# Superjie13/StereoTracking

Hardware: AMD Instinct MI355X
Metric: stereo frame-pairs/sec @1280x720 D=192 (higher is better)
Workload: dtype f32; 1 GPU; configs[1]: batch=8 synthetic 1280x720 stereo pairs per GPU, D=192, full YOLOX-s two-branch backbone+PAFPN+head, cost volume at 1/4 res (48 levels) + 2 3x3 aggregation convs + soft-argmin, decode+NMS, per-box depth; global_batch=8, inflight_contexts=4, distinct_input_batches=4, gpu_max_hw_queues=4, hip_force_dev_kernarg=1, parallelism=single process, no process group (no collective in the step), collectives_issued=0, tuning_plan=configs/tuning/mi355x.json, max_det=1000, detections_overflow=False

## Files before the change

include/stereotrack.h:

```cpp
#ifndef STEREOTRACK_H_
#define STEREOTRACK_H_

#include <stddef.h>
#include <stdint.h>

#ifdef __cplusplus
extern "C" {
#endif

#define ST_VERSION 430

enum {
  ST_OK = 0,
  ST_ERR_INVALID = -1,
  ST_ERR_HIP = -2,
  ST_ERR_STATE = -3,
  ST_ERR_WORKSPACE = -4,
  ST_ERR_NOTFOUND = -5
};

typedef void* st_stream_t;

int st_version(void);
const char* st_last_error(void);

typedef struct StConvDesc {
  const float* in_dev;
  int N, Hi, Wi, Cin, in_ld, in_off;
  const float* wgt_dev;
  const float* bias_dev;
  int Cout, KH, KW, stride, pad;
  float* out1_dev;
  int out1_ld, out1_off, split;
  float* out2_dev;
  int out2_ld, out2_off;
  float* up_dev;
  int up_ld, up_off;
  const float* res_dev;
  int res_ld, res_off;
  float post_scale;
  int act;
  const float* wgt_wino_dev;
} StConvDesc;

int st_conv2d_nhwc(const StConvDesc* d, st_stream_t stream);
int st_conv2d_nhwc_variant(const StConvDesc* d, st_stream_t stream, int variant);
size_t st_wino_packed_floats(int Cout, int Cin);
int st_wino_pack_weights(const float* packed_wgt_host, int Cout, int Cin, float* out_host);
int st_conv3x3_wino_group(const StConvDesc* descs, int n, st_stream_t stream);

int st_conv1x1_chain(const StConvDesc* a, const StConvDesc* b, st_stream_t stream);
size_t st_front_frag_floats(int Cout, int Cin);
int st_front_pack_frags(const float* packed_wgt_host, int Cout, int Cin, float* out_host);
int st_conv3x3s2_csp_front(const StConvDesc* a, const StConvDesc* ms, const StConvDesc* c1, const float* frag_ms_dev,
                           const float* frag_c1_dev, st_stream_t stream);
size_t st_csp_tail_frag_floats(void);
int st_csp_tail_pack_frags(const float* packed_wgt_host, float* out_host);
int st_conv3x3_csp_tail(const StConvDesc* conv2, const StConvDesc* fin, const float* frag_fin_dev, st_stream_t stream);
size_t st_conv_packed_floats(int Cout, int Cin, int KH, int KW);
int st_conv_pack_weights(const float* w, const float* conv_bias,
                         const float* bn_gamma, const float* bn_beta,
                         const float* bn_mean, const float* bn_var,
                         double bn_eps, int Cout, int Cin, int KH, int KW,
                         float* wgt_out, float* bias_out);

int st_focus_pack(const float* img_nchw_dev, int N, int C, int H, int W,
                  float* out_nhwc_dev, st_stream_t stream);

size_t st_stem_packed_floats(int Cout);
int st_stem_pack_weights(const float* w, const float* conv_bias,
                         const float* bn_gamma, const float* bn_beta,
                         const float* bn_mean, const float* bn_var,
                         double bn_eps, int Cout, int used_planes, float* wgt_out, float* bias_out);
int st_stem_focus_conv(const float* img_nchw_dev, int N, int H, int W, int used_planes, const float* wgt_dev,
                       const float* bias_dev, int Cout, float* out_nhwc_dev, int out_ld, int out_off,
                       int act , st_stream_t stream);
int st_stem_focus_conv_u8(const unsigned char* const* frames_u8_dev_ptrs_host, int N, int h, int w, int H, int W,
                          float pad_value, const float* wgt_dev, const float* bias_dev, int Cout, float* out_dev,
                          int out_ld, int out_off, int act, st_stream_t stream);

int st_pack_raw_inputs(const unsigned char* img_u8_dev, const unsigned short* disp_u16_dev, int N, int h, int w,
                       int H, int W, float img_pad, float* img_out_dev, float* disp_postp_out_dev,
                       float* disp_mask_out_dev, st_stream_t stream);
int st_pack_raw_frames(const unsigned char* const* frames_u8_dev_ptrs_host, int N, int h, int w, int H, int W,
                       float img_pad, float* img_out_dev, st_stream_t stream);
int st_resize_planes(const void* in_dev, int P, int h, int w, int interleaved, void* out_dev, int h2, int w2,
                     int elem_bytes, int bilinear, st_stream_t stream);

int st_spp_pool(const float* x_dev, int x_ld, int x_off, int N, int H, int W, int C,
                float* out_dev, int out_ld, int out_off, st_stream_t stream);

typedef struct StDetector StDetector;

typedef struct StDetectorConfig {
  int struct_size;
  float widen_factor;
  float deepen_factor;
  int num_classes;
  int batch;
// ... 398 lines not shown
```

stereotracking_amd/_lib.py:

```python
import ctypes as C
import os

import torch

_HERE = os.path.dirname(os.path.abspath(__file__))
LIB_PATH = os.path.join(_HERE, 'lib', 'libstereotrack_hip.so')

ST_OK = 0
_ERR_NAMES = {-1: 'ST_ERR_INVALID', -2: 'ST_ERR_HIP', -3: 'ST_ERR_STATE', -4: 'ST_ERR_WORKSPACE',
              -5: 'ST_ERR_NOTFOUND'}


class StError(RuntimeError):
    """A libstereotrack_hip call returned a non-zero status."""


class StConvDesc(C.Structure):
    _fields_ = [
        ('in_dev', C.c_void_p),
        ('N', C.c_int), ('Hi', C.c_int), ('Wi', C.c_int), ('Cin', C.c_int), ('in_ld', C.c_int), ('in_off', C.c_int),
        ('wgt_dev', C.c_void_p), ('bias_dev', C.c_void_p),
        ('Cout', C.c_int), ('KH', C.c_int), ('KW', C.c_int), ('stride', C.c_int), ('pad', C.c_int),
        ('out1_dev', C.c_void_p), ('out1_ld', C.c_int), ('out1_off', C.c_int), ('split', C.c_int),
        ('out2_dev', C.c_void_p), ('out2_ld', C.c_int), ('out2_off', C.c_int),
# ... 70 lines not shown
        [(n, C.c_void_p) for n in ('gt_rows', 'pred_rows', 'ignore_rows', 'frame_gt_off', 'frame_pred_off',
                                   'frame_ignore_off', 'frame_ws_off', 'class_table', 'ws')] + [('ws_bytes', C.c_size_t)] + \
        [(n, C.c_void_p) for n in ('gt_keep', 'pred_keep', 'status')]


class StTrackletArgs(C.Structure):
    _fields_ = [(n, C.c_int) for n in ('struct_size', 'num_rows', 'num_out_rows', 'num_tracks', 'first', 'count',
                                       'num_groups', 'max_rows')] + \
        [(n, C.c_void_p) for n in ('rows', 'row_out_off', 'row_gap', 'trk_out_off', 'trk_order', 'trk_len_scale', 'ws')] + \
        [('ws_bytes', C.c_size_t), ('out_rows', C.c_void_p), ('status', C.c_void_p), ('phase_ticks', C.c_void_p)]


class StStreamTick(C.Structure):
    _fields_ = [('struct_size', C.c_int), ('streams', C.c_int), ('chunk', C.c_int), ('num_chunks', C.c_int),
                ('max_dets', C.c_int), ('det_rows', C.c_int), ('stream_of_slot', C.c_void_p), ('frame_ids', C.c_void_p)]


class StHeadPredLevel(C.Structure):
    _fields_ = [('cls_dev', C.c_void_p), ('cls_ld', C.c_int), ('cls_off', C.c_int),
                ('reg_dev', C.c_void_p), ('reg_ld', C.c_int), ('reg_off', C.c_int),
                ('wgt_cls_dev', C.c_void_p), ('bias_cls_dev', C.c_void_p),
                ('wgt_reg_dev', C.c_void_p), ('bias_reg_dev', C.c_void_p),
                ('out_dev', C.c_void_p), ('M', C.c_int)]


class StDecodeDesc(C.Structure):
    _fields_ = [
        ('struct_size', C.c_int), ('batch', C.c_int), ('num_levels', C.c_int),
        ('level_h', C.c_int * 4), ('level_w', C.c_int * 4), ('level_stride', C.c_int * 4),
        ('level_offset', C.c_size_t * 4),
        ('score_thr', C.c_float), ('iou_thr', C.c_float), ('max_det', C.c_int),
        ('scale_x', C.c_float), ('scale_y', C.c_float), ('pad_left', C.c_float), ('pad_top', C.c_float),
        ('ori_w', C.c_float), ('ori_h', C.c_float), ('nms_mask_rows', C.c_int), ('num_classes', C.c_int),
        ('single_label', C.c_int),
    ]


_vp, _i, _f, _sz = C.c_void_p, C.c_int, C.c_float, C.c_size_t
_PROTOS = {
    'st_version': (C.c_int, []),
    'st_head_row_floats': (_i, [_i]),
    'st_png_unfilter': (_i, [_vp, _i, _i, _i, _vp]),
    'st_stem_focus_conv_u8': (_i, [_vp, _i, _i, _i, _i, _i, _f, _vp, _vp, _i, _vp, _i, _i, _i, _vp]),
    'st_detector_forward_raw': (_i, [_vp, _vp, _i, _i, _f, _vp, _vp, _sz, _vp, _vp]),
    'st_detector_forward_phase0_raw': (_i, [_vp, _vp, _vp, _i, _i, _f, _vp, _sz, _vp]),
    'st_pack_raw_frames': (_i, [_vp, _i, _i, _i, _i, _i, _f, _vp, _vp]),
    'st_resize_planes': (_i, [_vp, _i, _i, _i, _i, _vp, _i, _i, _i, _i, _vp]),
    'st_detector_set_split': (_i, [_vp, _i]),
    'st_split_instances_available': (_i, []),
    'st_volume_agg3d': (_i, [_vp, _vp, _i, _i, _i, _i, _vp, _f, _i, _vp]),
    'st_last_error': (C.c_char_p, []),
    'st_conv2d_nhwc': (_i, [C.POINTER(StConvDesc), _vp]),
    'st_conv2d_nhwc_variant': (_i, [C.POINTER(StConvDesc), _vp, _i]),
    'st_conv3x3_wino_group': (_i, [C.POINTER(StConvDesc), _i, _vp]),
    'st_head_pred': (_i, [C.POINTER(StHeadPredLevel), _i, _i, _vp]),
    'st_detector_op_owner': (_i, [_vp, _i, _vp, _vp]),
    'st_conv1x1_chain': (_i, [C.POINTER(StConvDesc), C.POINTER(StConvDesc), _vp]),
    'st_front_frag_floats': (_sz, [_i, _i]),
    'st_front_pack_frags': (_i, [_vp, _i, _i, _vp]),
    'st_conv3x3s2_csp_front': (_i, [C.POINTER(StConvDesc), C.POINTER(StConvDesc), C.POINTER(StConvDesc), _vp, _vp, _vp]),
    'st_csp_tail_frag_floats': (_sz, []),
    'st_csp_tail_pack_frags': (_i, [_vp, _vp]),
    'st_conv3x3_csp_tail': (_i, [C.POINTER(StConvDesc), C.POINTER(StConvDesc), _vp, _vp]),
    'st_conv_packed_floats': (_sz, [_i, _i, _i, _i]),
    'st_wino_packed_floats': (_sz, [_i, _i]),
    'st_wino_pack_weights': (_i, [_vp, _i, _i, _vp]),
    'st_conv_pack_weights': (_i, [_vp, _vp, _vp, _vp, _vp, _vp, C.c_double, _i, _i, _i, _i, _vp, _vp]),
    'st_focus_pack': (_i, [_vp, _i, _i, _i, _i, _vp, _vp]),
    'st_stem_packed_floats': (_sz, [_i]),
    'st_stem_pack_weights': (_i, [_vp, _vp, _vp, _vp, _vp, _vp, C.c_double, _i, _i, _vp, _vp]),
    'st_stem_focus_conv': (_i, [_vp, _i, _i, _i, _i, _vp, _vp, _i, _vp, _i, _i, _i, _vp]),
    'st_pack_raw_inputs': (_i, [_vp, _vp, _i, _i, _i, _i, _i, _f, _vp, _vp, _vp, _vp]),
    'st_spp_pool': (_i, [_vp, _i, _i, _i, _i, _i, _i, _vp, _i, _i, _vp]),
    'st_detector_create': (_i, [C.POINTER(StDetectorConfig), C.POINTER(_vp)]),
    'st_detector_destroy': (_i, [_vp]),
    'st_detector_num_params': (_i, [_vp]),
    'st_detector_param_info': (_i, [_vp, _i, C.c_char_p, _i, C.POINTER(C.c_int64), C.POINTER(_i)]),
    'st_detector_set_param': (_i, [_vp, C.c_char_p, _vp, C.c_int64]),
    'st_detector_finalize': (_i, [_vp]),
    'st_detector_workspace_bytes': (_sz, [_vp]),
    'st_detector_head_floats': (_sz, [_vp]),
    'st_detector_num_levels': (_i, [_vp]),
    'st_detector_level_info': (_i, [_vp, _i, C.POINTER(_i), C.POINTER(_i), C.POINTER(_i), C.POINTER(_sz)]),
    'st_detector_forward': (_i, [_vp, _vp, _vp, _vp, _sz, _vp, _vp]),
    'st_detector_forward_phase': (_i, [_vp, _i, _vp, _vp, _vp, _vp, _sz, _vp, _vp]),
    'st_detector_macs': (C.c_double, [_vp]),
    'st_detector_set_timing': (_i, [_vp, _i]),
    'st_detector_num_ops': (_i, [_vp]),
    'st_detector_op_times': (_i, [_vp, _i, _vp, _vp, _vp, _vp, _vp]),
    'st_detector_autotune': (_i, [_vp, _vp, _sz, _vp, _vp, _i]),
    'st_conv_variant_name': (C.c_char_p, [_i]),
    'st_conv_variant_signature': (C.c_char_p, [_i]),
    'st_detector_get_tuning': (_i, [_vp, _vp, _i]),
    'st_detector_set_tuning': (_i, [_vp, _vp, _i]),
    'st_detector_op_desc': (_i, [_vp, _i, C.c_char_p, _i]),
    'st_detector_tap': (_i, [_vp, C.c_char_p, _vp, C.POINTER(_vp), C.POINTER(_i), C.POINTER(_i),
                             C.POINTER(_i), C.POINTER(_i), C.POINTER(_i)]),
    'st_decode_nms_workspace_bytes': (_sz, [C.POINTER(StDecodeDesc)]),
    'st_lapjv_extended': (_i, [_vp, _i, _i, C.c_double, _vp, _vp]),
    'st_tracker_create': (_i, [C.POINTER(StTrackerConfig), C.POINTER(_vp)]),
    'st_tracker_destroy': (_i, [_vp]),
    'st_tracker_reset': (_i, [_vp]),
    'st_tracker_track': (_i, [_vp, _i, _vp, _i, _vp, _vp, _i, C.POINTER(_i)]),
    'st_tracker_track_records': (_i, [_vp, _vp, _vp, _i, _i, _i, _vp, _vp, _i, _vp]),
    'st_tracker_cmc_needed': (_i, [_vp, _i, _i]),
    'st_tracker_track_cmc': (_i, [_vp, _i, _vp, _i, _vp, _vp, _vp, _i, C.POINTER(_i)]),
# ... 102 lines not shown
```

stereotracking_amd/csrc/conv_igemm.hip:

```cpp
#include <algorithm>

#include <type_traits>

#include "st_common.h"

namespace st {

typedef float f32x16 __attribute__((ext_vector_type(16)));
typedef float f32x4 __attribute__((ext_vector_type(4)));
typedef unsigned int u32x4 __attribute__((ext_vector_type(4)));

struct ConvKArgs {
  const float* in;
  const float* wgt;
  const float* bias;
  float* out1;
  float* out2;
  float* up;
  const float* res;
  int Hi, Wi, Cin, in_ld, in_off;
  int Ho, Wo, HoWo, Cout;
  int KH, KW, stride, pad;
  int K, Kpad, M;
  unsigned in_bytes, wgt_bytes;
  int out1_ld, out1_off, split;
  int out2_ld, out2_off;
  int up_ld, up_off;
  int res_ld, res_off;
  float post_scale;
  int act;
  int n_tiles;
};

constexpr int BK = 32;
constexpr int LDK = 36;

__device__ __forceinline__ float silu_f32(float v) {
  return v * __builtin_amdgcn_rcpf(1.0f + __expf(-v));
}

template <int TM, int TN>
__device__ __forceinline__ void conv_epilogue(const ConvKArgs& p, f32x16 (&acc)[TM][TN], int m0, int n0, int wm,
                                              int wn, int l31, int lh, int BM, int BN) {
  const bool full_tile = (m0 + BM <= p.M) && (n0 + BN <= p.Cout);
  const bool side1 = !p.out2 || n0 + BN <= p.split, side2 = p.out2 && n0 >= p.split;
  const bool simple = full_tile && !p.up && (side1 || side2);
  if (simple) {
    float* __restrict__ o1 = side1 ? p.out1 + p.out1_off : p.out2 + p.out2_off - p.split;
    const unsigned o_ld = side1 ? (unsigned)p.out1_ld : (unsigned)p.out2_ld;
    const float* __restrict__ rs = p.res ? p.res + p.res_off : nullptr;
#pragma unroll
    for (int tj = 0; tj < TN; ++tj) {
      const unsigned j = n0 + wn * 32 * TN + tj * 32 + l31;
// ... 24 lines not shown
    const float bj = p.bias[j];
    const bool vj = j < p.Cout;
#pragma unroll
    for (int ti = 0; ti < TM; ++ti) {
      float rv[16];
      if (p.res) {
#pragma unroll
        for (int r = 0; r < 16; ++r) {
          const int m = m0 + wm * 32 * TM + ti * 32 + (r & 3) + 8 * (r >> 2) + 4 * lh;
          rv[r] = (m < p.M && vj) ? p.res[(unsigned)m * (unsigned)p.res_ld + p.res_off + j] : 0.f;
        }
      }
      int un = 0, uy = 0, ux = 0;
      if (p.up) {
        const int mfirst = m0 + wm * 32 * TM + ti * 32 + 4 * lh;
        un = mfirst / p.HoWo;
        const int rem = mfirst - un * p.HoWo;
        uy = rem / p.Wo;
        ux = rem - uy * p.Wo;
      }
#pragma unroll
      for (int r = 0; r < 16; ++r) {
        const int m = m0 + wm * 32 * TM + ti * 32 + (r & 3) + 8 * (r >> 2) + 4 * lh;
        if (p.up && r > 0) {
          ux += (r & 3) ? 1 : 5;
          while (ux >= p.Wo) {
            ux -= p.Wo;
            if (++uy == p.Ho) { uy = 0; ++un; }
          }
        }
        if (m < p.M && vj) {
          float v = acc[ti][tj][r] + bj;
          if (p.act) v = silu_f32(v);
          if (p.res) v = (v + rv[r]) * p.post_scale;
          if (j < p.split)
            p.out1[(unsigned)m * (unsigned)p.out1_ld + p.out1_off + j] = v;
          else
            p.out2[(unsigned)m * (unsigned)p.out2_ld + p.out2_off + (j - p.split)] = v;
          if (p.up) {
            const unsigned W2 = 2u * p.Wo;
            const unsigned base = ((unsigned)un * 2u * p.Ho + 2u * uy) * W2 + 2u * ux;
            float* u = p.up + p.up_off + j;
            u[base * (unsigned)p.up_ld] = v;
            u[(base + 1) * (unsigned)p.up_ld] = v;
            u[(base + W2) * (unsigned)p.up_ld] = v;
            u[(base + W2 + 1) * (unsigned)p.up_ld] = v;
          }
        }
      }
    }
  }
}

template <int TM, int TN, int WM, int WN, int NBUF, int ILV = 1, int DMA = 0, int PW = 0>
__global__ __launch_bounds__(64 * WM * WN) void conv_igemm_kernel(ConvKArgs p) {
  static_assert(NBUF == 2 || (WM == 1 && WN == 1), "single LDS buffer needs a single-wave block");
  static_assert(!DMA || (NBUF == 2 && 64 * WM * WN >= 128), "LDS-DMA variant: double buffer, >= 2 waves");
  constexpr int LDK = DMA ? 32 : st::LDK;
  constexpr int NT = 64 * WM * WN;
  constexpr int BM = 32 * TM * WM;
  constexpr int BN = 32 * TN * WN;
  constexpr int ROWS = NT / 8;
  constexpr int AP = BM / ROWS;
  constexpr int BP = BN / ROWS;
  static_assert(BM % ROWS == 0 && BN % ROWS == 0, "tile/thread mismatch");

  extern __shared__ __attribute__((aligned(16))) float smem[];
  float* As = smem;
  float* Bs = smem + NBUF * BM * LDK;

  const int nblk = gridDim.x, bid = blockIdx.x;
  const int q = nblk >> 3, r8 = nblk & 7, xcd = bid & 7, slot = bid >> 3;
  const int logical = (xcd < r8 ? xcd * (q + 1) : r8 * (q + 1) + (xcd - r8) * q) + slot;
  const int mt = logical / p.n_tiles;
  const int nt = logical - mt * p.n_tiles;
  const int m0 = mt * BM, n0 = nt * BN;

  const int tid = threadIdx.x;
  const int lane = tid & 63, wave = tid >> 6;
  const int wm = wave / WN, wn = wave - wm * WN;
  const int l31 = lane & 31, lh = lane >> 5;

  const int r0 = tid >> 3;
  const int kq = DMA ? ((tid & 7) ^ ((r0 >> 1) & 7)) : (tid & 7);
  const __amdgpu_buffer_rsrc_t rsrcA =
      __builtin_amdgcn_make_buffer_rsrc(const_cast<float*>(p.in), 0, p.in_bytes, 0x00020000);
  const __amdgpu_buffer_rsrc_t rsrcB =
      __builtin_amdgcn_make_buffer_rsrc(const_cast<float*>(p.wgt), 0, p.wgt_bytes, 0x00020000);
  int rowoff[AP];
  unsigned vmask[AP];
#pragma unroll
  for (int a = 0; a < AP; ++a) {
    const int m = m0 + r0 + a * ROWS;
    const bool vm = m < p.M;
    const int mm = vm ? m : 0;
    if (PW) {
      rowoff[a] = (mm * p.in_ld + p.in_off) * 4;
      vmask[a] = vm ? 1u : 0u;
      continue;
    }
    const int n = mm / p.HoWo;
    const int rem = mm - n * p.HoWo;
    const int oy = rem / p.Wo;
    const int ox = rem - oy * p.Wo;
    const int iy0 = oy * p.stride - p.pad, ix0 = ox * p.stride - p.pad;
    rowoff[a] = (((n * p.Hi + iy0) * p.Wi + ix0) * p.in_ld + p.in_off) * 4;
    unsigned msk = 0;
    for (int kh = 0; kh < p.KH; ++kh)
      for (int kw = 0; kw < p.KW; ++kw)
        if (vm && (unsigned)(iy0 + kh) < (unsigned)p.Hi && (unsigned)(ix0 + kw) < (unsigned)p.Wi)
          msk |= 1u << (kh * p.KW + kw);
    vmask[a] = msk;
  }
  unsigned woff[BP];
#pragma unroll
  for (int b = 0; b < BP; ++b) woff[b] = ((unsigned)(n0 + r0 + b * ROWS) * (unsigned)p.Kpad + kq * 4) * 4u;

  int kc_c = kq * 4, kc_kh = 0, kc_kw = 0, kc_k = kq * 4;
  if (!PW) {
    while (kc_c >= p.Cin) {
      kc_c -= p.Cin;
      if (++kc_kw == p.KW) { kc_kw = 0; ++kc_kh; }
    }
  }
  int kc_tap = PW ? 0 : kc_kh * p.KW + kc_kw;
  int kc_off = PW ? kc_k * 4 : ((kc_kh * p.Wi + kc_kw) * p.in_ld + kc_c) * 4;

  f32x4 areg[AP], breg[BP];
  auto load_a = [&](int a, bool vk) {
    const bool v = vk && ((vmask[a] >> kc_tap) & 1u);
    const unsigned off = v ? (unsigned)(rowoff[a] + kc_off) : 0x80000000u;
    areg[a] = __builtin_bit_cast(f32x4, __builtin_amdgcn_raw_buffer_load_b128(rsrcA, off, 0, 0));
  };
  auto load_b = [&](int b, int kc) {
    breg[b] = __builtin_bit_cast(
        f32x4, __builtin_amdgcn_raw_buffer_load_b128(rsrcB, woff[b], kc * (BK * 4), 0));
  };
  auto advance = [&]() {
    kc_k += BK;
    if (PW) {
      kc_off += BK * 4;
      return;
    }
    kc_c += BK;
    while (kc_c >= p.Cin) {
      kc_c -= p.Cin;
      if (++kc_kw == p.KW) { kc_kw = 0; ++kc_kh; }
    }
    kc_tap = kc_kh * p.KW + kc_kw;
    kc_off = ((kc_kh * p.Wi + kc_kw) * p.in_ld + kc_c) * 4;
  };
  auto store_a = [&](int a, int buf) {
    *reinterpret_cast<f32x4*>(As + buf * BM * LDK + (r0 + a * ROWS) * LDK + kq * 4) = areg[a];
  };
  auto store_b = [&](int b, int buf) {
    *reinterpret_cast<f32x4*>(Bs + buf * BN * LDK + (r0 + b * ROWS) * LDK + kq * 4) = breg[b];
  };
  auto dma_a = [&](int a, bool vk, int buf) {
    const bool v = vk && ((vmask[a] >> kc_tap) & 1u);
    const unsigned off = v ? (unsigned)(rowoff[a] + kc_off) : 0x80000000u;
#if defined(__HIP_DEVICE_COMPILE__)
    __builtin_amdgcn_raw_ptr_buffer_load_lds(
        rsrcA, (__attribute__((address_space(3))) void*)(As + buf * BM * LDK + (wave * 8 + a * ROWS) * LDK), 16, off,
        0, 0, 0);
#else
    (void)off; (void)buf;
#endif
  };
  auto dma_b = [&](int b, int kc, int buf) {
#if defined(__HIP_DEVICE_COMPILE__)
    __builtin_amdgcn_raw_ptr_buffer_load_lds(
        rsrcB, (__attribute__((address_space(3))) void*)(Bs + buf * BN * LDK + (wave * 8 + b * ROWS) * LDK), 16,
        woff[b], kc * (BK * 4), 0, 0);
#else
    (void)b; (void)kc; (void)buf;
#endif
  };
  auto dma_chunk = [&](int kc, int buf) {
    const bool vk = kc_k < p.K;
#pragma unroll
    for (int a = 0; a < AP; ++a) dma_a(a, vk, buf);
#pragma unroll
    for (int b = 0; b < BP; ++b) dma_b(b, kc, buf);
    advance();
  };
  auto load_chunk = [&](int kc) {
    const bool vk = kc_k < p.K;
#pragma unroll
    for (int a = 0; a < AP; ++a) load_a(a, vk);
#pragma unroll
    for (int b = 0; b < BP; ++b) load_b(b, kc);
    advance();
  };
  auto store_chunk = [&](int buf) {
#pragma unroll
    for (int a = 0; a < AP; ++a) store_a(a, buf);
#pragma unroll
    for (int b = 0; b < BP; ++b) store_b(b, buf);
  };

  f32x16 acc[TM][TN];
#pragma unroll
  for (int i = 0; i < TM; ++i)
#pragma unroll
    for (int j = 0; j < TN; ++j)
#pragma unroll
      for (int r = 0; r < 16; ++r) acc[i][j][r] = 0.f;

  const int nchunks = p.Kpad / BK;
  if (DMA) {
    dma_chunk(0, 0);
  } else {
    load_chunk(0);
    store_chunk(0);
  }
  if (DMA) asm volatile("s_waitcnt vmcnt(0)" ::: "memory");
  __syncthreads();

  constexpr int NI = AP + BP;
  auto do_chunk = [&](int kc, auto more_tag) {
    constexpr bool MORE = decltype(more_tag)::value;
    const int buf = NBUF == 2 ? (kc & 1) : 0;
    const int nbuf = NBUF == 2 ? (buf ^ 1) : 0;
    constexpr bool more = MORE;
    const bool vk = kc_k < p.K;
    if (!DMA && !ILV && more) load_chunk(kc + 1);
    if (DMA && !ILV && more) dma_chunk(kc + 1, nbuf);

    const float* Ab = As + buf * BM * LDK + (wm * 32 * TM + l31) * LDK + (DMA ? 0 : 4 * lh);
    const float* Bb = Bs + buf * BN * LDK + (wn * 32 * TN + l31) * LDK + (DMA ? 0 : 4 * lh);
    const int sw = (l31 >> 1) & 7;
    const int gmax = MORE ? 4 : (p.K - kc * BK + 7) >> 3;
    f32x4 a[2][TM], b[2][TN];
    auto read_frags = [&](int g, int set) {
      const int koff = DMA ? (((2 * g + lh) ^ sw) * 4) : g * 8;
#pragma unroll
      for (int i = 0; i < TM; ++i)
        a[set][i] = *reinterpret_cast<const f32x4*>(Ab + i * 32 * LDK + koff);
#pragma unroll
      for (int j = 0; j < TN; ++j)
        b[set][j] = *reinterpret_cast<const f32x4*>(Bb + j * 32 * LDK + koff);
    };
    read_frags(0, 0);
#pragma unroll
    for (int g = 0; g < 4; ++g) {
      if (!MORE && g >= gmax) break;
      const int set = g & 1;
      if (g + 1 < 4) read_frags(g + 1, set ^ 1);
      __builtin_amdgcn_sched_barrier(0);
#pragma unroll
      for (int s = 0; s < 4; ++s) {
#pragma unroll
        for (int i = 0; i < TM; ++i)
#pragma unroll
          for (int j = 0; j < TN; ++j)
            acc[i][j] = __builtin_amdgcn_mfma_f32_32x32x2f32(a[set][i][s], b[set][j][s], acc[i][j], 0, 0, 0);
        if (DMA && ILV) {
          const int slot = g * 4 + s;
          if (more) {
#pragma unroll
            for (int it = 0; it < NI; ++it) {
              if ((it * 8) / NI == slot) {
                if (it < AP) dma_a(it, vk, nbuf); else dma_b(it - AP, kc + 1, nbuf);
              }
            }
            if (slot == 7) advance();
          }
        }
        if (!DMA && ILV && NBUF == 2) {
          const int slot = g * 4 + s;
          if (more) {
#pragma unroll
            for (int it = 0; it < NI; ++it) {
              if ((it * 8) / NI == slot) {
                if (it < AP) load_a(it, vk); else load_b(it - AP, kc + 1);
              }
              if (8 + (it * 8) / NI == slot) {
                if (it < AP) store_a(it, nbuf); else store_b(it - AP, nbuf);
              }
            }
            if (slot == 7) advance();
          }
        }
      }
    }

    if (!DMA && (!ILV || NBUF != 2) && more) {
      if (ILV) load_chunk(kc + 1);
      store_chunk(nbuf);
    }
    if (DMA) asm volatile("s_waitcnt vmcnt(0)" ::: "memory");
    __syncthreads();
  };
  for (int kc = 0; kc + 1 < nchunks; ++kc) do_chunk(kc, std::true_type{});
  do_chunk(nchunks - 1, std::false_type{});

  conv_epilogue<TM, TN>(p, acc, m0, n0, wm, wn, l31, lh, BM, BN);
}

#ifdef ST_ABLATION
typedef __bf16 bf16x8 __attribute__((ext_vector_type(8)));

typedef unsigned u32x2 __attribute__((ext_vector_type(2)));
__device__ __forceinline__ unsigned sp_cvt_pk_bf16(float lo, float hi) {
  unsigned r;
  asm("v_cvt_pk_bf16_f32 %0, %1, %2" : "=v"(r) : "v"(lo), "v"(hi));
  return r;
}
__device__ __forceinline__ float sp_lo_f32(unsigned pk) { return __builtin_bit_cast(float, pk << 16); }
__device__ __forceinline__ float sp_hi_f32(unsigned pk) { return __builtin_bit_cast(float, pk & 0xFFFF0000u); }
__device__ __forceinline__ void split3_f32x4(const f32x4 x, u32x2& hi, u32x2& mid, u32x2& lo) {
#pragma unroll
  for (int e = 0; e < 2; ++e) {
    const float x0 = x[2 * e], x1 = x[2 * e + 1];
    const unsigned h = sp_cvt_pk_bf16(x0, x1);
    const float r0 = x0 - sp_lo_f32(h), r1 = x1 - sp_hi_f32(h);
    const unsigned m = sp_cvt_pk_bf16(r0, r1);
    const float q0 = r0 - sp_lo_f32(m), q1 = r1 - sp_hi_f32(m);
    hi[e] = h; mid[e] = m; lo[e] = sp_cvt_pk_bf16(q0, q1);
  }
}

template <int TM, int TN, int WM, int WN, int PW, int SBK, bool SACC>
__global__ __launch_bounds__(64 * WM * WN, (SBK == 16 ? 2 : 1)) void conv_split_kernel(ConvKArgs p) {
  constexpr int NT = 64 * WM * WN;
  constexpr int BM = 32 * TM * WM;
  constexpr int BN = 32 * TN * WN;
  constexpr int KQ = SBK / 4;
  constexpr int SP_LDK = SBK + 8;
  constexpr int NSTEP = SBK / 16;
  constexpr int ROWS = NT / KQ;
  constexpr int AP = BM / ROWS;
  constexpr int BP = BN / ROWS;
  static_assert(BM % ROWS == 0 && BN % ROWS == 0, "tile/thread mismatch");
  extern __shared__ __attribute__((aligned(16))) float smem[];
  __bf16* As = reinterpret_cast<__bf16*>(smem);
  __bf16* Bs = As + 3 * BM * SP_LDK;

  const int nblk = gridDim.x, bid = blockIdx.x;
  const int q = nblk >> 3, r8 = nblk & 7, xcd = bid & 7, slot = bid >> 3;
  const int logical = (xcd < r8 ? xcd * (q + 1) : r8 * (q + 1) + (xcd - r8) * q) + slot;
  const int mt = logical / p.n_tiles;
  const int nt = logical - mt * p.n_tiles;
  const int m0 = mt * BM, n0 = nt * BN;

  const int tid = threadIdx.x;
  const int lane = tid & 63, wave = tid >> 6;
  const int wm = wave / WN, wn = wave - wm * WN;
// ... 168 lines not shown
    }
    __syncthreads();
  };
  using T = std::true_type;
  using F = std::false_type;
  using S0 = std::integral_constant<int, 0>;
  using S1 = std::integral_constant<int, 1>;
  int kc = 0;
  for (; kc + 3 < nchunks; kc += 2) {
    do_chunk(kc, S0{}, T{}, T{});
    do_chunk(kc + 1, S1{}, T{}, T{});
  }
  for (; kc < nchunks; ++kc) {
    const bool m1 = kc + 1 < nchunks, m2 = kc + 2 < nchunks;
    if (kc & 1) {
      if (m2) do_chunk(kc, S1{}, T{}, T{}); else if (m1) do_chunk(kc, S1{}, T{}, F{}); else do_chunk(kc, S1{}, F{}, F{});
    } else {
      if (m2) do_chunk(kc, S0{}, T{}, T{}); else if (m1) do_chunk(kc, S0{}, T{}, F{}); else do_chunk(kc, S0{}, F{}, F{});
    }
  }
  if (SACC) {
#pragma unroll
    for (int i = 0; i < TM; ++i)
#pragma unroll
      for (int j = 0; j < TN; ++j) acc[i][j] += accS[SACC ? i : 0][SACC ? j : 0];
  }
  conv_epilogue<TM, TN>(p, acc, m0, n0, wm, wn, l31, lh, BM, BN);
}

template <int TM, int TN, int WM, int WN, int PW, int SBK>
static int launch_split(const ConvKArgs& a, int m_tiles, hipStream_t stream) {
  constexpr int BM = 32 * TM * WM, BN = 32 * TN * WN;
  constexpr size_t lds = (size_t)2 * 3 * (BM + BN) * (SBK + 8) * 2;
  static bool attr_set = false;
  constexpr bool SACC = !(TM == 2 && TN == 2 && SBK == 16);
  auto kern = conv_split_kernel<TM, TN, WM, WN, PW, SBK, SACC>;
  if (!attr_set) {
    ST_CHECK_HIP(hipFuncSetAttribute(reinterpret_cast<const void*>(kern),
                                     hipFuncAttributeMaxDynamicSharedMemorySize, (int)lds));
    attr_set = true;
  }
  dim3 grid((unsigned)(m_tiles * a.n_tiles)), block(64 * WM * WN);
  hipLaunchKernelGGL(kern, grid, block, lds, stream, a);
  ST_CHECK_HIP(hipGetLastError());
  return ST_OK;
}

#endif

#ifdef ST_ABLATION
#include "experiments/conv_igemm_ws.inc"
#endif

template <int TM, int TN, int WM, int WN, int NBUF = 2, int ILV = 1, int DMA = 0, int PW = 0>
static int launch_variant(const ConvKArgs& a, int m_tiles, hipStream_t stream) {
  constexpr int BM = 32 * TM * WM, BN = 32 * TN * WN;
  constexpr size_t lds = (size_t)NBUF * (BM + BN) * (DMA ? 32 : LDK) * sizeof(float);
  static bool attr_set = false;
  auto kern = conv_igemm_kernel<TM, TN, WM, WN, NBUF, ILV, DMA, PW>;
  if (!attr_set) {
    ST_CHECK_HIP(hipFuncSetAttribute(reinterpret_cast<const void*>(kern),
                                     hipFuncAttributeMaxDynamicSharedMemorySize, (int)lds));
    attr_set = true;
  }
  dim3 grid((unsigned)(m_tiles * a.n_tiles)), block(64 * WM * WN);
  hipLaunchKernelGGL(kern, grid, block, lds, stream, a);
  ST_CHECK_HIP(hipGetLastError());
  return ST_OK;
}

struct ConvVariant { int bm, bn, threads; };
static const ConvVariant kVariants[] = {{128, 128, 256}, {128, 64, 128}, {128, 32, 128}, {64, 64, 256},
                                        {64, 32, 128},   {128, 64, 256}, {128, 32, 256}, {64, 128, 256},
                                        {256, 64, 256},  {64, 64, 64},   {64, 32, 64},   {32, 64, 64},
                                        {128, 128, 256}, {64, 64, 256},  {64, 128, 256}, {128, 32, 256},
                                        {128, 64, 256},  {128, 128, 256}, {64, 64, 256},
                                        {256, 128, 512}, {256, 128, 512}, {256, 128, 512},
                                        {128, 128, 320}, {64, 64, 320},   {64, 128, 320}, {128, 32, 320},
                                        {128, 64, 320},  {128, 128, 384}, {64, 128, 384}, {128, 128, 512}};
#ifdef ST_ABLATION
constexpr int kNumVariants = 30;
#else
constexpr int kNumVariants = 22;
#endif

int conv_variant_count() { return kNumVariants; }
bool conv_variant_valid(int id, int cout) {
  return id >= 0 && id < kNumVariants && round_up(cout, 32) % kVariants[id].bn == 0;
}
const char* conv_variant_name(int id) {
  static const char* names[] = {"128x128", "128x64w2", "128x32w2", "64x64", "64x32w2",
                                "128x64", "128x32", "64x128", "256x64", "64x64w1", "64x32w1", "32x64w1",
                                "128x128dma", "64x64dma", "64x128dma", "128x32dma", "128x64dma",
                                "128x128dmab", "64x64dmab", "256x128dma", "256x128dmab", "256x128",
                                "128x128ws", "64x64ws", "64x128ws", "128x32ws", "128x64ws", "128x128ws2",
                                "64x128ws2", "128x128ws4"};
  return id >= 0 && id < kNumVariants ? names[id] : "-";
}

const char* conv_variant_signature(int id) {
  static const char* sigs[] = {"2, 2, 2, 2, 2, 1, 0", "2, 2, 2, 1, 2, 1, 0", "2, 1, 2, 1, 2, 1, 0",
                               "1, 1, 2, 2, 2, 1, 0", "1, 1, 2, 1, 2, 1, 0", "1, 2, 4, 1, 2, 1, 0",
                               "1, 1, 4, 1, 2, 1, 0", "1, 2, 2, 2, 2, 1, 0", "2, 2, 4, 1, 2, 1, 0",
                               "2, 2, 1, 1, 1, 1, 0", "2, 1, 1, 1, 1, 1, 0", "1, 2, 1, 1, 1, 1, 0",
                               "2, 2, 2, 2, 2, 1, 1", "1, 1, 2, 2, 2, 1, 1", "1, 2, 2, 2, 2, 1, 1",
                               "1, 1, 4, 1, 2, 1, 1", "1, 2, 4, 1, 2, 1, 1", "2, 2, 2, 2, 2, 0, 1",
                               "1, 1, 2, 2, 2, 0, 1", "2, 2, 4, 2, 2, 1, 1", "2, 2, 4, 2, 2, 0, 1",
                               "2, 2, 4, 2, 2, 1, 0", "ws 2, 2, 2, 2", "ws 1, 1, 2, 2", "ws 1, 2, 2, 2",
                               "ws 1, 1, 4, 1", "ws 1, 2, 4, 1", "ws 2, 2, 2, 2, 2", "ws 1, 2, 2, 2, 2",
                               "ws 2, 2, 2, 2, 4"};
  return id >= 0 && id < kNumVariants ? sigs[id] : "";
}

bool pw_conv_applicable(const StConvDesc& d);
int pw_conv_launch(const StConvDesc& d, hipStream_t stream, const StConvDesc* chain);
int pwr_conv_launch(const StConvDesc& d, hipStream_t stream, const StConvDesc* chain);
bool pwr_chain_applicable(const StConvDesc& d, const StConvDesc& c);
bool dc_conv_applicable(const StConvDesc& d);
int dc_conv_launch(const StConvDesc& d, hipStream_t stream);
bool wino_conv_applicable(const StConvDesc& d);
int wino_conv_launch(const StConvDesc& d, hipStream_t stream, bool narrow);
// ... 61 lines not shown
  a.out1_ld = d.out1_ld; a.out1_off = d.out1_off; a.split = split;
  a.out2_ld = d.out2_ld; a.out2_off = d.out2_off;
  a.up_ld = d.up_ld; a.up_off = d.up_off;
  a.res_ld = d.res_ld; a.res_off = d.res_off;
  a.post_scale = d.res_dev ? d.post_scale : 1.0f;
  a.act = d.act;

  const int cout_pad = round_up(d.Cout, 32);
  if (force_variant >= 50 && force_variant <= 55) {
    static const int sbm[3] = {128, 64, 128}, sbn[3] = {128, 64, 64};
    const int vi = (force_variant - 50) % 3, k16 = (force_variant - 50) / 3;
    ST_REQUIRE(cout_pad % sbn[vi] == 0, "conv: split variant %d does not divide Cout=%d", force_variant, d.Cout);
#ifndef ST_ABLATION
    (void)sbm; (void)k16;
    return set_error(ST_ERR_INVALID, "conv: the split-operand (bf16x3) instances 50-55 are parked in the tools-only build "
                                     "(make ABLATION=1, ST_LIBRARY=...libstereotrack_hip_ablation.so)");
#else
    if (picked_variant) *picked_variant = force_variant;
    a.n_tiles = cout_pad / sbn[vi];
    const int m_tiles = ceil_div(a.M, sbm[vi]);
    const bool pw = d.KH == 1 && d.KW == 1 && d.stride == 1 && d.pad == 0;
    switch (vi + 3 * k16) {
      case 0: return pw ? launch_split<2, 2, 2, 2, 1, 32>(a, m_tiles, stream) : launch_split<2, 2, 2, 2, 0, 32>(a, m_tiles, stream);
      case 1: return pw ? launch_split<1, 1, 2, 2, 1, 32>(a, m_tiles, stream) : launch_split<1, 1, 2, 2, 0, 32>(a, m_tiles, stream);
      case 2: return pw ? launch_split<1, 2, 4, 1, 1, 32>(a, m_tiles, stream) : launch_split<1, 2, 4, 1, 0, 32>(a, m_tiles, stream);
      case 3: return pw ? launch_split<2, 2, 2, 2, 1, 16>(a, m_tiles, stream) : launch_split<2, 2, 2, 2, 0, 16>(a, m_tiles, stream);
      case 4: return pw ? launch_split<1, 1, 2, 2, 1, 16>(a, m_tiles, stream) : launch_split<1, 1, 2, 2, 0, 16>(a, m_tiles, stream);
      default: return pw ? launch_split<1, 2, 4, 1, 1, 16>(a, m_tiles, stream) : launch_split<1, 2, 4, 1, 0, 16>(a, m_tiles, stream);
    }
#endif
  }
  int pick = -1;
  if (force_variant >= 0) {
    ST_REQUIRE(conv_variant_valid(force_variant % 100, d.Cout), "conv: variant %d does not divide Cout=%d",
               force_variant, d.Cout);
    pick = force_variant % 100;
  } else {
    static const int order[] = {0, 5, 6, 3, 4};
    long long best_blocks = -1;
    for (int id : order) {
      if (!conv_variant_valid(id, d.Cout)) continue;
      const long long blocks = (long long)ceil_div(a.M, kVariants[id].bm) * (cout_pad / kVariants[id].bn);
      if (blocks >= 512) { pick = id; break; }
      if (blocks > best_blocks) { best_blocks = blocks; pick = id; }
    }
  }
  const ConvVariant& v = kVariants[pick];
  if (picked_variant) *picked_variant = pick;
  a.n_tiles = cout_pad / v.bn;
  const int m_tiles = ceil_div(a.M, v.bm);
  ST_REQUIRE(force_variant < 100, "conv: no such instance %d", force_variant);
  const bool pw = d.KH == 1 && d.KW == 1 && d.stride == 1 && d.pad == 0;
  switch (pick) {
    case 0: return pw ? launch_variant<2, 2, 2, 2, 2, 1, 0, 1>(a, m_tiles, stream) : launch_variant<2, 2, 2, 2, 2, 1, 0, 0>(a, m_tiles, stream);
    case 1: return pw ? launch_variant<2, 2, 2, 1, 2, 1, 0, 1>(a, m_tiles, stream) : launch_variant<2, 2, 2, 1, 2, 1, 0, 0>(a, m_tiles, stream);
    case 2: return pw ? launch_variant<2, 1, 2, 1, 2, 1, 0, 1>(a, m_tiles, stream) : launch_variant<2, 1, 2, 1, 2, 1, 0, 0>(a, m_tiles, stream);
    case 3: return pw ? launch_variant<1, 1, 2, 2, 2, 1, 0, 1>(a, m_tiles, stream) : launch_variant<1, 1, 2, 2, 2, 1, 0, 0>(a, m_tiles, stream);
    case 4: return pw ? launch_variant<1, 1, 2, 1, 2, 1, 0, 1>(a, m_tiles, stream) : launch_variant<1, 1, 2, 1, 2, 1, 0, 0>(a, m_tiles, stream);
    case 5: return pw ? launch_variant<1, 2, 4, 1, 2, 1, 0, 1>(a, m_tiles, stream) : launch_variant<1, 2, 4, 1, 2, 1, 0, 0>(a, m_tiles, stream);
    case 6: return pw ? launch_variant<1, 1, 4, 1, 2, 1, 0, 1>(a, m_tiles, stream) : launch_variant<1, 1, 4, 1, 2, 1, 0, 0>(a, m_tiles, stream);
    case 7: return pw ? launch_variant<1, 2, 2, 2, 2, 1, 0, 1>(a, m_tiles, stream) : launch_variant<1, 2, 2, 2, 2, 1, 0, 0>(a, m_tiles, stream);
    case 8: return pw ? launch_variant<2, 2, 4, 1, 2, 1, 0, 1>(a, m_tiles, stream) : launch_variant<2, 2, 4, 1, 2, 1, 0, 0>(a, m_tiles, stream);
    case 9: return pw ? launch_variant<2, 2, 1, 1, 1, 1, 0, 1>(a, m_tiles, stream) : launch_variant<2, 2, 1, 1, 1, 1, 0, 0>(a, m_tiles, stream);
    case 10: return pw ? launch_variant<2, 1, 1, 1, 1, 1, 0, 1>(a, m_tiles, stream) : launch_variant<2, 1, 1, 1, 1, 1, 0, 0>(a, m_tiles, stream);
    case 11: return pw ? launch_variant<1, 2, 1, 1, 1, 1, 0, 1>(a, m_tiles, stream) : launch_variant<1, 2, 1, 1, 1, 1, 0, 0>(a, m_tiles, stream);
    case 12: return pw ? launch_variant<2, 2, 2, 2, 2, 1, 1, 1>(a, m_tiles, stream) : launch_variant<2, 2, 2, 2, 2, 1, 1, 0>(a, m_tiles, stream);
    case 13: return pw ? launch_variant<1, 1, 2, 2, 2, 1, 1, 1>(a, m_tiles, stream) : launch_variant<1, 1, 2, 2, 2, 1, 1, 0>(a, m_tiles, stream);
    case 14: return pw ? launch_variant<1, 2, 2, 2, 2, 1, 1, 1>(a, m_tiles, stream) : launch_variant<1, 2, 2, 2, 2, 1, 1, 0>(a, m_tiles, stream);
    case 15: return pw ? launch_variant<1, 1, 4, 1, 2, 1, 1, 1>(a, m_tiles, stream) : launch_variant<1, 1, 4, 1, 2, 1, 1, 0>(a, m_tiles, stream);
    case 16: return pw ? launch_variant<1, 2, 4, 1, 2, 1, 1, 1>(a, m_tiles, stream) : launch_variant<1, 2, 4, 1, 2, 1, 1, 0>(a, m_tiles, stream);
    case 17: return pw ? launch_variant<2, 2, 2, 2, 2, 0, 1, 1>(a, m_tiles, stream) : launch_variant<2, 2, 2, 2, 2, 0, 1, 0>(a, m_tiles, stream);
    case 18: return pw ? launch_variant<1, 1, 2, 2, 2, 0, 1, 1>(a, m_tiles, stream) : launch_variant<1, 1, 2, 2, 2, 0, 1, 0>(a, m_tiles, stream);
    case 19: return pw ? launch_variant<2, 2, 4, 2, 2, 1, 1, 1>(a, m_tiles, stream) : launch_variant<2, 2, 4, 2, 2, 1, 1, 0>(a, m_tiles, stream);
    case 20: return pw ? launch_variant<2, 2, 4, 2, 2, 0, 1, 1>(a, m_tiles, stream) : launch_variant<2, 2, 4, 2, 2, 0, 1, 0>(a, m_tiles, stream);
    case 21: return pw ? launch_variant<2, 2, 4, 2, 2, 1, 0, 1>(a, m_tiles, stream) : launch_variant<2, 2, 4, 2, 2, 1, 0, 0>(a, m_tiles, stream);
#ifdef ST_ABLATION
    case 22: return launch_ws<2, 2, 2, 2>(a, m_tiles, stream);
    case 23: return launch_ws<1, 1, 2, 2>(a, m_tiles, stream);
    case 24: return launch_ws<1, 2, 2, 2>(a, m_tiles, stream);
    case 25: return launch_ws<1, 1, 4, 1>(a, m_tiles, stream);
    case 26: return launch_ws<1, 2, 4, 1>(a, m_tiles, stream);
    case 27: return launch_ws<2, 2, 2, 2, 2>(a, m_tiles, stream);
    case 28: return launch_ws<1, 2, 2, 2, 2>(a, m_tiles, stream);
    case 29: return launch_ws<2, 2, 2, 2, 4>(a, m_tiles, stream);
#endif
    default: return set_error(ST_ERR_INVALID, "conv: unknown tile variant %d", pick);
  }
}

}

extern "C" int st_conv2d_nhwc(const StConvDesc* d, st_stream_t stream) {
  if (!d) return st::set_error(ST_ERR_INVALID, "st_conv2d_nhwc: null desc");
  return st::conv2d_launch(*d, static_cast<hipStream_t>(stream), -1, nullptr);
}

extern "C" int st_conv1x1_chain(const StConvDesc* a, const StConvDesc* b, st_stream_t stream) {
  if (!a || !b) return st::set_error(ST_ERR_INVALID, "st_conv1x1_chain: null desc");
  if (st::pwr_chain_applicable(*a, *b)) return st::pwr_conv_launch(*a, static_cast<hipStream_t>(stream), b);
  return st::pw_conv_launch(*a, static_cast<hipStream_t>(stream), b);
}

extern "C" int st_conv2d_nhwc_variant(const StConvDesc* d, st_stream_t stream, int variant) {
  if (!d) return st::set_error(ST_ERR_INVALID, "st_conv2d_nhwc_variant: null desc");
  return st::conv2d_launch(*d, static_cast<hipStream_t>(stream), variant, nullptr);
}
```

Measured before the change: 1754 stereo frame-pairs/s.

## Add deeper register-staged prefetch distance to interleaved implicit-GEMM conv kernels

Adds a staging-distance template parameter to the register-staged, double-buffered igemm conv kernel so global loads are issued one or two K-chunks ahead, using two register sets when the distance is two. The main loop is unrolled over alternating register sets, with tail handling for the remaining chunks. Tile variants 1-8 and 21 now use distance 2 (distance 1 for some pointwise variants), and a legacy switch can turn it off. The aim is to hide global-memory latency behind MFMA work, at the cost of extra VGPRs, which may lower occupancy or cause spills.

Measured after the change: 1757 stereo frame-pairs/s, median of 6. About the same (+0.1%).

```diff
diff --git a/include/stereotrack.h b/include/stereotrack.h
--- a/include/stereotrack.h
+++ b/include/stereotrack.h
@@ -45,6 +45,7 @@
 
 int st_conv2d_nhwc(const StConvDesc* d, st_stream_t stream);
 int st_conv2d_nhwc_variant(const StConvDesc* d, st_stream_t stream, int variant);
+void st_conv_set_legacy_staging(int on);
 size_t st_wino_packed_floats(int Cout, int Cin);
 int st_wino_pack_weights(const float* packed_wgt_host, int Cout, int Cin, float* out_host);
 int st_conv3x3_wino_group(const StConvDesc* descs, int n, st_stream_t stream);
diff --git a/stereotracking_amd/_lib.py b/stereotracking_amd/_lib.py
--- a/stereotracking_amd/_lib.py
+++ b/stereotracking_amd/_lib.py
@@ -146,6 +146,7 @@
     'st_last_error': (C.c_char_p, []),
     'st_conv2d_nhwc': (_i, [C.POINTER(StConvDesc), _vp]),
     'st_conv2d_nhwc_variant': (_i, [C.POINTER(StConvDesc), _vp, _i]),
+    'st_conv_set_legacy_staging': (None, [_i]),
     'st_conv3x3_wino_group': (_i, [C.POINTER(StConvDesc), _i, _vp]),
     'st_head_pred': (_i, [C.POINTER(StHeadPredLevel), _i, _i, _vp]),
     'st_detector_op_owner': (_i, [_vp, _i, _vp, _vp]),
diff --git a/stereotracking_amd/csrc/conv_igemm.hip b/stereotracking_amd/csrc/conv_igemm.hip
--- a/stereotracking_amd/csrc/conv_igemm.hip
+++ b/stereotracking_amd/csrc/conv_igemm.hip
@@ -1,4 +1,5 @@
 #include <algorithm>
+#include <cstdlib>
 
 #include <type_traits>
 
@@ -129,9 +130,10 @@
   }
 }
 
-template <int TM, int TN, int WM, int WN, int NBUF, int ILV = 1, int DMA = 0, int PW = 0>
+template <int TM, int TN, int WM, int WN, int NBUF, int ILV = 1, int DMA = 0, int PW = 0, int SD = 0>
 __global__ __launch_bounds__(64 * WM * WN) void conv_igemm_kernel(ConvKArgs p) {
   static_assert(NBUF == 2 || (WM == 1 && WN == 1), "single LDS buffer needs a single-wave block");
+  static_assert(SD == 0 || (SD <= 2 && !DMA && ILV && NBUF == 2), "staging distance: register-staged interleaved instances");
   static_assert(!DMA || (NBUF == 2 && 64 * WM * WN >= 128), "LDS-DMA variant: double buffer, >= 2 waves");
   constexpr int LDK = DMA ? 32 : st::LDK;
   constexpr int NT = 64 * WM * WN;
@@ -203,14 +205,15 @@
   int kc_tap = PW ? 0 : kc_kh * p.KW + kc_kw;
   int kc_off = PW ? kc_k * 4 : ((kc_kh * p.Wi + kc_kw) * p.in_ld + kc_c) * 4;
 
-  f32x4 areg[AP], breg[BP];
-  auto load_a = [&](int a, bool vk) {
+  constexpr int NSET = SD == 2 ? 2 : 1;
+  f32x4 areg[NSET][AP], breg[NSET][BP];
+  auto load_a = [&](int a, bool vk, int set = 0) {
     const bool v = vk && ((vmask[a] >> kc_tap) & 1u);
     const unsigned off = v ? (unsigned)(rowoff[a] + kc_off) : 0x80000000u;
-    areg[a] = __builtin_bit_cast(f32x4, __builtin_amdgcn_raw_buffer_load_b128(rsrcA, off, 0, 0));
-  };
-  auto load_b = [&](int b, int kc) {
-    breg[b] = __builtin_bit_cast(
+    areg[set][a] = __builtin_bit_cast(f32x4, __builtin_amdgcn_raw_buffer_load_b128(rsrcA, off, 0, 0));
+  };
+  auto load_b = [&](int b, int kc, int set = 0) {
+    breg[set][b] = __builtin_bit_cast(
         f32x4, __builtin_amdgcn_raw_buffer_load_b128(rsrcB, woff[b], kc * (BK * 4), 0));
   };
   auto advance = [&]() {
@@ -227,11 +230,11 @@
     kc_tap = kc_kh * p.KW + kc_kw;
     kc_off = ((kc_kh * p.Wi + kc_kw) * p.in_ld + kc_c) * 4;
   };
-  auto store_a = [&](int a, int buf) {
-    *reinterpret_cast<f32x4*>(As + buf * BM * LDK + (r0 + a * ROWS) * LDK + kq * 4) = areg[a];
-  };
-  auto store_b = [&](int b, int buf) {
-    *reinterpret_cast<f32x4*>(Bs + buf * BN * LDK + (r0 + b * ROWS) * LDK + kq * 4) = breg[b];
+  auto store_a = [&](int a, int buf, int set = 0) {
+    *reinterpret_cast<f32x4*>(As + buf * BM * LDK + (r0 + a * ROWS) * LDK + kq * 4) = areg[set][a];
+  };
+  auto store_b = [&](int b, int buf, int set = 0) {
+    *reinterpret_cast<f32x4*>(Bs + buf * BN * LDK + (r0 + b * ROWS) * LDK + kq * 4) = breg[set][b];
   };
   auto dma_a = [&](int a, bool vk, int buf) {
     const bool v = vk && ((vmask[a] >> kc_tap) & 1u);
@@ -261,19 +264,19 @@
     for (int b = 0; b < BP; ++b) dma_b(b, kc, buf);
     advance();
   };
-  auto load_chunk = [&](int kc) {
+  auto load_chunk = [&](int kc, int set = 0) {
     const bool vk = kc_k < p.K;
 #pragma unroll
-    for (int a = 0; a < AP; ++a) load_a(a, vk);
-#pragma unroll
-    for (int b = 0; b < BP; ++b) load_b(b, kc);
+    for (int a = 0; a < AP; ++a) load_a(a, vk, set);
+#pragma unroll
+    for (int b = 0; b < BP; ++b) load_b(b, kc, set);
     advance();
   };
-  auto store_chunk = [&](int buf) {
-#pragma unroll
-    for (int a = 0; a < AP; ++a) store_a(a, buf);
-#pragma unroll
-    for (int b = 0; b < BP; ++b) store_b(b, buf);
+  auto store_chunk = [&](int buf, int set = 0) {
+#pragma unroll
+    for (int a = 0; a < AP; ++a) store_a(a, buf, set);
+#pragma unroll
+    for (int b = 0; b < BP; ++b) store_b(b, buf, set);
   };
 
   f32x16 acc[TM][TN];
@@ -287,17 +290,26 @@
   const int nchunks = p.Kpad / BK;
   if (DMA) {
     dma_chunk(0, 0);
+  } else if (SD == 2) {
+    load_chunk(0, 0);
+    if (nchunks > 1) load_chunk(1, 1);
+    store_chunk(0, 0);
+    if (nchunks > 2) load_chunk(2, 0);
   } else {
     load_chunk(0);
     store_chunk(0);
+    if (SD == 1 && nchunks > 1) load_chunk(1);
   }
   if (DMA) asm volatile("s_waitcnt vmcnt(0)" ::: "memory");
   __syncthreads();
 
   constexpr int NI = AP + BP;
-  auto do_chunk = [&](int kc, auto more_tag) {
+  static_assert(NI <= 16, "one staging item per MFMA slot");
+  auto do_chunk = [&](int kc, auto more_tag, auto load_tag, auto set_tag) __attribute__((always_inline)) {
     constexpr bool MORE = decltype(more_tag)::value;
-    const int buf = NBUF == 2 ? (kc & 1) : 0;
+    constexpr bool LOAD = decltype(load_tag)::value;
+    constexpr int SET = decltype(set_tag)::value;
+    const int buf = NBUF == 2 ? (SD == 2 && MORE ? (SET ^ 1) : (kc & 1)) : 0;
     const int nbuf = NBUF == 2 ? (buf ^ 1) : 0;
     constexpr bool more = MORE;
     const bool vk = kc_k < p.K;
@@ -344,7 +356,21 @@
             if (slot == 7) advance();
           }
         }
-        if (!DMA && ILV && NBUF == 2) {
+        if (SD > 0) {
+          const int slot = g * 4 + s;
+#pragma unroll
+          for (int it = 0; it < NI; ++it) {
+            if ((it * 16) / NI != slot) continue;
+            if (MORE) {
+              if (it < AP) store_a(it, nbuf, SET); else store_b(it - AP, nbuf, SET);
+            }
+            if (LOAD) {
+              if (it < AP) load_a(it, vk, SET); else load_b(it - AP, kc + 1 + SD, SET);
+            }
+          }
+          if (LOAD && slot == ((NI - 1) * 16) / NI) advance();
+        }
+        if (!DMA && ILV && NBUF == 2 && SD == 0) {
           const int slot = g * 4 + s;
           if (more) {
 #pragma unroll
@@ -369,8 +395,30 @@
     if (DMA) asm volatile("s_waitcnt vmcnt(0)" ::: "memory");
     __syncthreads();
   };
-  for (int kc = 0; kc + 1 < nchunks; ++kc) do_chunk(kc, std::true_type{});
-  do_chunk(nchunks - 1, std::false_type{});
+  using T = std::true_type;
+  using F = std::false_type;
+  using S0 = std::integral_constant<int, 0>;
+  using S1 = std::integral_constant<int, 1>;
+  if constexpr (SD == 0) {
+    for (int kc = 0; kc + 1 < nchunks; ++kc) do_chunk(kc, T{}, T{}, S0{});
+    do_chunk(nchunks - 1, F{}, F{}, S0{});
+  } else if constexpr (SD == 1) {
+    int kc = 0;
+    for (; kc + 2 < nchunks; ++kc) do_chunk(kc, T{}, T{}, S0{});
+    if (kc + 1 < nchunks) { do_chunk(kc, T{}, F{}, S0{}); ++kc; }
+    do_chunk(kc, F{}, F{}, S0{});
+  } else {
+    int kc = 0;
+    for (; kc + 4 < nchunks; kc += 2) {
+      do_chunk(kc, T{}, T{}, S1{});
+      do_chunk(kc + 1, T{}, T{}, S0{});
+    }
+    int left = nchunks - kc;
+    if (left == 4) { do_chunk(kc, T{}, T{}, S1{}); do_chunk(kc + 1, T{}, F{}, S0{}); kc += 2; left = 2; }
+    if (left == 3) { do_chunk(kc, T{}, F{}, S1{}); do_chunk(kc + 1, T{}, F{}, S0{}); kc += 2; left = 1; }
+    if (left == 2) { do_chunk(kc, T{}, F{}, S1{}); ++kc; }
+    do_chunk(kc, F{}, F{}, S0{});
+  }
 
   conv_epilogue<TM, TN>(p, acc, m0, n0, wm, wn, l31, lh, BM, BN);
 }
@@ -645,12 +693,12 @@
 #include "experiments/conv_igemm_ws.inc"
 #endif
 
-template <int TM, int TN, int WM, int WN, int NBUF = 2, int ILV = 1, int DMA = 0, int PW = 0>
+template <int TM, int TN, int WM, int WN, int NBUF = 2, int ILV = 1, int DMA = 0, int PW = 0, int SD = 0>
 static int launch_variant(const ConvKArgs& a, int m_tiles, hipStream_t stream) {
   constexpr int BM = 32 * TM * WM, BN = 32 * TN * WN;
   constexpr size_t lds = (size_t)NBUF * (BM + BN) * (DMA ? 32 : LDK) * sizeof(float);
   static bool attr_set = false;
-  auto kern = conv_igemm_kernel<TM, TN, WM, WN, NBUF, ILV, DMA, PW>;
+  auto kern = conv_igemm_kernel<TM, TN, WM, WN, NBUF, ILV, DMA, PW, SD>;
   if (!attr_set) {
     ST_CHECK_HIP(hipFuncSetAttribute(reinterpret_cast<const void*>(kern),
                                      hipFuncAttributeMaxDynamicSharedMemorySize, (int)lds));
@@ -660,6 +708,22 @@
   hipLaunchKernelGGL(kern, grid, block, lds, stream, a);
   ST_CHECK_HIP(hipGetLastError());
   return ST_OK;
+}
+
+static int g_legacy_staging = 0;
+
+template <int TM, int TN, int WM, int WN, int PW, int SDP>
+static int launch_staged(const ConvKArgs& a, int m_tiles, hipStream_t stream) {
+  int sd = g_legacy_staging ? 0 : SDP;
+#ifdef ST_ABLATION
+  static const int env_sd = [] { const char* e = getenv("ST_CONV_SD"); return e ? atoi(e) : -1; }();
+  if (!g_legacy_staging && env_sd >= 0 && env_sd <= 2) sd = env_sd;
+  if (sd == 2) return launch_variant<TM, TN, WM, WN, 2, 1, 0, PW, 2>(a, m_tiles, stream);
+  if (sd == 1) return launch_variant<TM, TN, WM, WN, 2, 1, 0, PW, 1>(a, m_tiles, stream);
+#else
+  if (sd != 0) return launch_variant<TM, TN, WM, WN, 2, 1, 0, PW, SDP>(a, m_tiles, stream);
+#endif
+  return launch_variant<TM, TN, WM, WN, 2, 1, 0, PW, 0>(a, m_tiles, stream);
 }
 
 struct ConvVariant { int bm, bn, threads; };
@@ -827,15 +891,15 @@
   ST_REQUIRE(force_variant < 100, "conv: no such instance %d", force_variant);
   const bool pw = d.KH == 1 && d.KW == 1 && d.stride == 1 && d.pad == 0;
   switch (pick) {
-    case 0: return pw ? launch_variant<2, 2, 2, 2, 2, 1, 0, 1>(a, m_tiles, stream) : launch_variant<2, 2, 2, 2, 2, 1, 0, 0>(a, m_tiles, stream);
-    case 1: return pw ? launch_variant<2, 2, 2, 1, 2, 1, 0, 1>(a, m_tiles, stream) : launch_variant<2, 2, 2, 1, 2, 1, 0, 0>(a, m_tiles, stream);
-    case 2: return pw ? launch_variant<2, 1, 2, 1, 2, 1, 0, 1>(a, m_tiles, stream) : launch_variant<2, 1, 2, 1, 2, 1, 0, 0>(a, m_tiles, stream);
-    case 3: return pw ? launch_variant<1, 1, 2, 2, 2, 1, 0, 1>(a, m_tiles, stream) : launch_variant<1, 1, 2, 2, 2, 1, 0, 0>(a, m_tiles, stream);
-    case 4: return pw ? launch_variant<1, 1, 2, 1, 2, 1, 0, 1>(a, m_tiles, stream) : launch_variant<1, 1, 2, 1, 2, 1, 0, 0>(a, m_tiles, stream);
-    case 5: return pw ? launch_variant<1, 2, 4, 1, 2, 1, 0, 1>(a, m_tiles, stream) : launch_variant<1, 2, 4, 1, 2, 1, 0, 0>(a, m_tiles, stream);
-    case 6: return pw ? launch_variant<1, 1, 4, 1, 2, 1, 0, 1>(a, m_tiles, stream) : launch_variant<1, 1, 4, 1, 2, 1, 0, 0>(a, m_tiles, stream);
-    case 7: return pw ? launch_variant<1, 2, 2, 2, 2, 1, 0, 1>(a, m_tiles, stream) : launch_variant<1, 2, 2, 2, 2, 1, 0, 0>(a, m_tiles, stream);
-    case 8: return pw ? launch_variant<2, 2, 4, 1, 2, 1, 0, 1>(a, m_tiles, stream) : launch_variant<2, 2, 4, 1, 2, 1, 0, 0>(a, m_tiles, stream);
+    case 0: return pw ? launch_staged<2, 2, 2, 2, 1, 0>(a, m_tiles, stream) : launch_staged<2, 2, 2, 2, 0, 0>(a, m_tiles, stream);
+    case 1: return pw ? launch_staged<2, 2, 2, 1, 1, 2>(a, m_tiles, stream) : launch_staged<2, 2, 2, 1, 0, 2>(a, m_tiles, stream);
+    case 2: return pw ? launch_staged<2, 1, 2, 1, 1, 2>(a, m_tiles, stream) : launch_staged<2, 1, 2, 1, 0, 2>(a, m_tiles, stream);
+    case 3: return pw ? launch_staged<1, 1, 2, 2, 1, 1>(a, m_tiles, stream) : launch_staged<1, 1, 2, 2, 0, 2>(a, m_tiles, stream);
+    case 4: return pw ? launch_staged<1, 1, 2, 1, 1, 2>(a, m_tiles, stream) : launch_staged<1, 1, 2, 1, 0, 2>(a, m_tiles, stream);
+    case 5: return pw ? launch_staged<1, 2, 4, 1, 1, 2>(a, m_tiles, stream) : launch_staged<1, 2, 4, 1, 0, 2>(a, m_tiles, stream);
+    case 6: return pw ? launch_staged<1, 1, 4, 1, 1, 2>(a, m_tiles, stream) : launch_staged<1, 1, 4, 1, 0, 2>(a, m_tiles, stream);
+    case 7: return pw ? launch_staged<1, 2, 2, 2, 1, 1>(a, m_tiles, stream) : launch_staged<1, 2, 2, 2, 0, 2>(a, m_tiles, stream);
+    case 8: return pw ? launch_staged<2, 2, 4, 1, 1, 2>(a, m_tiles, stream) : launch_staged<2, 2, 4, 1, 0, 2>(a, m_tiles, stream);
     case 9: return pw ? launch_variant<2, 2, 1, 1, 1, 1, 0, 1>(a, m_tiles, stream) : launch_variant<2, 2, 1, 1, 1, 1, 0, 0>(a, m_tiles, stream);
     case 10: return pw ? launch_variant<2, 1, 1, 1, 1, 1, 0, 1>(a, m_tiles, stream) : launch_variant<2, 1, 1, 1, 1, 1, 0, 0>(a, m_tiles, stream);
     case 11: return pw ? launch_variant<1, 2, 1, 1, 1, 1, 0, 1>(a, m_tiles, stream) : launch_variant<1, 2, 1, 1, 1, 1, 0, 0>(a, m_tiles, stream);
@@ -848,7 +912,7 @@
     case 18: return pw ? launch_variant<1, 1, 2, 2, 2, 0, 1, 1>(a, m_tiles, stream) : launch_variant<1, 1, 2, 2, 2, 0, 1, 0>(a, m_tiles, stream);
     case 19: return pw ? launch_variant<2, 2, 4, 2, 2, 1, 1, 1>(a, m_tiles, stream) : launch_variant<2, 2, 4, 2, 2, 1, 1, 0>(a, m_tiles, stream);
     case 20: return pw ? launch_variant<2, 2, 4, 2, 2, 0, 1, 1>(a, m_tiles, stream) : launch_variant<2, 2, 4, 2, 2, 0, 1, 0>(a, m_tiles, stream);
-    case 21: return pw ? launch_variant<2, 2, 4, 2, 2, 1, 0, 1>(a, m_tiles, stream) : launch_variant<2, 2, 4, 2, 2, 1, 0, 0>(a, m_tiles, stream);
+    case 21: return pw ? launch_staged<2, 2, 4, 2, 1, 2>(a, m_tiles, stream) : launch_staged<2, 2, 4, 2, 0, 2>(a, m_tiles, stream);
 #ifdef ST_ABLATION
     case 22: return launch_ws<2, 2, 2, 2>(a, m_tiles, stream);
     case 23: return launch_ws<1, 1, 2, 2>(a, m_tiles, stream);
@@ -865,6 +929,8 @@
 
 }
 
+extern "C" void st_conv_set_legacy_staging(int on) { st::g_legacy_staging = on != 0; }
+
 extern "C" int st_conv2d_nhwc(const StConvDesc* d, st_stream_t stream) {
   if (!d) return st::set_error(ST_ERR_INVALID, "st_conv2d_nhwc: null desc");
   return st::conv2d_launch(*d, static_cast<hipStream_t>(stream), -1, nullptr);
```
